# HKUST-Aerial-Robotics/FUEL

Hardware: AMD Instinct MI355X
Metric: plan_cycles_per_sec (higher is better)
Workload: dtype u64 bit-planes / u16 (u32 beyond 255 voxels) exact squared distances / f32 ESDF / f64 log-odds and B-spline

## Files before the change

fuel_amd/_lib.py:

```python
import ctypes as C
import os

_HERE = os.path.dirname(os.path.abspath(__file__))
LIB_PATH = os.environ.get("FUELMI_LIB_PATH") or os.path.join(_HERE, "libfuelmi.so")
_LIB = None

K_INFLATE, K_ESDF_ZY, K_ESDF_X, K_FRONTIER, K_BSPLINE, K_INSERT, K_COUNT = range(7)


class FuelmiError(RuntimeError):
    pass


class MapCfg(C.Structure):
    _fields_ = [
        ("resolution", C.c_double),
        ("map_size", C.c_double * 3),
        ("ground_height", C.c_double),
        ("obstacles_inflation", C.c_double),
        ("local_bound_inflate", C.c_double),
        ("default_dist", C.c_double),
        ("optimistic", C.c_int),
        ("signed_dist", C.c_int),
        ("p_hit", C.c_double),
# ... 264 lines not shown
    "fuelmi_map_get_updated_box": (C.c_int, [_P, _dp, _dp, C.c_int]),
    "fuelmi_map_set_updated_box": (C.c_int, [_P, _dp, _dp]),
    "fuelmi_map_upload_occupancy": (C.c_int, [_P, _dp]),
    "fuelmi_map_sync_host": (C.c_int, [_P, _ip, _ip, _dp, C.c_void_p, _dp]),
    "fuelmi_map_register_mirrors": (C.c_int, [_P, _dp, C.c_void_p, _dp]),
    "fuelmi_map_unregister_mirrors": (C.c_int, [_P]),
    "fuelmi_map_dist_grad": (C.c_int, [_P, _dp, C.c_int, _dp, _dp]),
    "fuelmi_map_coarse_dist": (C.c_int, [_P, _dp, C.c_int, _dp]),
    "fuelmi_map_query_state": (C.c_int, [_P, _ip, C.c_int, _ip, _ip]),
    "fuelmi_map_synchronize": (C.c_int, [_P]),
    "fuelmi_frontier_set_viewpoint_cfg": (C.c_int, [_P, C.POINTER(ViewpointCfg)]),
    "fuelmi_frontier_compute_to_visit": (C.c_int, [_P, C.POINTER(C.c_int), C.POINTER(C.c_int)]),
    "fuelmi_frontier_viewpoint_count": (C.c_int, [_P, C.c_int, C.c_int]),
    "fuelmi_frontier_viewpoints": (C.c_int, [_P, C.c_int, C.c_int, _dp, C.POINTER(C.c_int)]),
    "fuelmi_frontier_is_covered": (C.c_int, [_P, C.POINTER(C.c_int)]),
    "fuelmi_frontier_cluster_filtered_size": (C.c_int, [_P, C.c_int, C.c_int]),
    "fuelmi_frontier_cluster_filtered": (C.c_int, [_P, C.c_int, C.c_int, C.c_void_p]),
    "fuelmi_frontier_create": (C.c_int, [_P, C.POINTER(FrontierCfg), _PP]),
    "fuelmi_frontier_destroy": (None, [_P]),
    "fuelmi_frontier_reset": (C.c_int, [_P]),
    "fuelmi_frontier_stats": (C.c_int, [_P, C.POINTER(C.c_int)]),
    "fuelmi_frontier_resolved_in_launch": (C.c_int, [_P]),
    "fuelmi_frontier_path_stats": (C.c_int, [_P, C.POINTER(C.c_int)]),
    "fuelmi_frontier_changed_stats": (C.c_int, [_P, C.POINTER(C.c_int)]),
    "fuelmi_frontier_order_stats": (C.c_int, [_P, C.POINTER(C.c_int)]),
    "fuelmi_frontier_synchronize": (C.c_int, [_P]),
    "fuelmi_bench_cycles": (C.c_int, [_P, _P, _P, _dp, _dp, C.c_int, C.c_int, C.POINTER(C.c_int), _dp]),
    "fuelmi_bench_host_profile": (C.c_int, [_P, _dp]),
    "fuelmi_bench_cycles_delivered": (C.c_int, [_P, _P, _P, _dp, _dp, C.c_int, _ip, C.c_size_t, _dp, _dp,
                                                C.POINTER(C.c_int), _dp]),
    "fuelmi_bench_stream": (C.c_int, [_P, _P, _P, C.c_int, C.POINTER(C.c_void_p), C.c_int, C.c_int, C.POINTER(DepthCfg),
                                      _dp, _dp, C.c_int, C.POINTER(C.c_int), _dp, _dp]),
    "fuelmi_frontier_search": (C.c_int, [_P, _ip]),
    "fuelmi_frontier_search_begin": (C.c_int, [_P]),
    "fuelmi_frontier_search_end": (C.c_int, [_P, _ip]),
    "fuelmi_frontier_keep_previous": (C.c_int, [_P, C.c_int]),
    "fuelmi_frontier_commit": (C.c_int, [_P, C.c_int]),
    "fuelmi_frontier_count": (C.c_int, [_P, C.c_int]),
    "fuelmi_frontier_cluster_size": (C.c_int, [_P, C.c_int, C.c_int]),
    "fuelmi_frontier_cluster_cells": (C.c_int, [_P, C.c_int, C.c_int, _ip]),
    "fuelmi_frontier_cluster_centres": (C.c_int, [_P, C.c_int, C.c_int, _dp]),
    "fuelmi_frontier_cluster_info": (C.c_int, [_P, C.c_int, C.c_int, _dp]),
    "fuelmi_frontier_removed_count": (C.c_int, [_P]),
    "fuelmi_frontier_removed_ids": (C.c_int, [_P, _ip]),
    "fuelmi_frontier_get_flags": (C.c_int, [_P, C.c_void_p]),
    "fuelmi_map_path_costs": (C.c_int, [_P, C.POINTER(PathCfg), C.c_int, _dp, _dp, _dp, _ip, _ip, _dp]),
# ... 110 lines not shown
```

fuel_amd/csrc/frontier.hip:

```cpp
#include <algorithm>
#include <chrono>
#include <cmath>
#include <cstdlib>
#include <cstring>
#include <list>
#include <memory>
#include <vector>

#include "fuelmi_internal.h"
#include "frontier_internal.h"

__global__ void k_zero_words(u64* p, int n) {
  for (int i = blockIdx.x * blockDim.x + threadIdx.x; i < n; i += gridDim.x * blockDim.x) p[i] = 0ull;
}

template <typename T>
static int dmalloc(fuelmi_frontier* f, T** p, size_t n) {
  void* d = nullptr;
  HIPCHK(hipMalloc(&d, std::max<size_t>(n, 1) * sizeof(T)));
  f->allocs.push_back(d);
  *p = (T*)d;
  const char* fp = reinterpret_cast<const char*>(p), *f0 = reinterpret_cast<const char*>(&f->F);
  if (fp >= f0 && fp < f0 + sizeof(FArgs))
    f->f_scratch.push_back({(size_t)(fp - f0), std::max<size_t>(n, 1) * sizeof(T)});
// ... 209 lines not shown
  F.h_counts = reinterpret_cast<u32*>(f->h_pin);
  F.h_rec = reinterpret_cast<KeptRec*>(F.h_counts + 16);
  F.h_part = reinterpret_cast<u32*>(F.h_rec + F.cap_kept);
  F.h_cells = F.h_part + ((size_t)F.cap_q / SZ_CH + 2) * 10;
  F.hcells_direct_max = FR_HCELLS_DIRECT;
  f->TY = 16;
  f->TX = std::max(1, std::min(8, (48 * 1024) / (f->TY * g.nz * 4)));
  const int qx = F.qbox.hi[0] - F.qbox.lo[0] + 1, qy = F.qbox.hi[1] - F.qbox.lo[1] + 1;
  f->ccl_tiles = 0;
  if (qx > 0 && qy > 0 && F.qbox.lo[2] <= F.qbox.hi[2]) {
    const int TX = f->TX, TY = f->TY;
    const int ntx = (qx + TX - 1) / TX, nty = (qy + TY - 1) / TY;
    f->ccl_tiles = ntx * nty;
    f->ccl_lds = ((size_t)TX * TY * g.nz + 2 * (size_t)TX * TY * ((g.nz + 31) / 32) + 2 * (size_t)TX) * sizeof(u32);
    if (f->ccl_lds > 160 * 1024) {
      fuelmi_set_error("frontier CCL tile of %d z-lines x %d voxels does not fit the LDS", TX * TY, g.nz);
      fuelmi_frontier_destroy(f);
      return FUELMI_ELIMIT;
    }
    if ((rc = frontier_legacy_attrs(f))) return rc;
    const int mtx = 4, mty = 8;
    f->fast_tiles = ((qx + 1 + mtx - 1) / mtx) * ((qy + 1 + mty - 1) / mty);
    F.pm_stride = (qx + 1 + mtx - 1) / mtx;
    if ((rc = dmalloc(f, &F.vlab, (size_t)g.N + 64)) || (rc = dmalloc(f, &F.tlab, (size_t)f->fast_tiles * FR_TCELL)) ||
        (rc = dmalloc(f, &F.t_base, (size_t)f->fast_tiles)) || (rc = dmalloc(f, &F.t_nroots, (size_t)f->fast_tiles)) ||
        (rc = dmalloc(f, &F.pm, (size_t)FR_KCAP * F.pm_stride))) {
      fuelmi_frontier_destroy(f);
      return rc;
    }
    const size_t seg_words = frontier_tile_lds(f, qx, qy);
    if ((rc = dmalloc(f, &F.tq, seg_words + 64)) || (rc = dmalloc(f, &F.ts, seg_words + 64))) {
      fuelmi_frontier_destroy(f);
      return rc;
    }
  }
  if ((rc = frontier_tile_attrs(f))) return rc;
  f->fast_ok = f->ccl_tiles > 0 && cfg->cluster_min >= 1 && frontier_tile_fits(f) && getenv("FUELMI_FRONTIER_LEGACY") == nullptr;
  if ((rc = frontier_twin_set(f))) {
    fuelmi_frontier_destroy(f);
    return rc;
  }
  {
    std::lock_guard<std::mutex> lk(m->dep_mu);
    m->dependents.push_back({f, &frontier_orphan});
  }
  *out = f;
  return FUELMI_OK;
}

int frontier_materialize_lists(fuelmi_frontier* f) {
  if (!f->lazy_kept) return FUELMI_OK;
  for (std::list<HCluster>* L : {&f->frontiers, &f->dormant})
    for (HCluster& c : *L)
      if (c.lazy) {
// ... 640 lines not shown
```

fuel_amd/csrc/frontier_internal.h:

```cpp
#ifndef FUELMI_FRONTIER_INTERNAL_H_
#define FUELMI_FRONTIER_INTERNAL_H_

#include <algorithm>
#include <chrono>
#include <cstring>
#include <list>
#include <memory>
#include <vector>

#include "fuelmi_internal.h"

#define NOCLAIM 0xFFFFFFFFu
#define SZ_CH 1024

struct KeptRec {
  u32 addr, slot, size, off;
  unsigned long long sum[3];
  u32 box[6];
  u32 pad[2];
};

struct FVar {
  Box3 sbox;
  int w0;
// ... 52 lines not shown
  u32* parent;
  u32* claim;
  int* cell_slot;
  u32* seed_adr;
  u32* csize;
  u32* kept;
  u32 cap_kept;
  int* slot2rank;
  struct KeptRec* krec;
  u32* ms_key[2];
  u32* ms_val[2];
  u32* ms_hist;
  u32 ms_nb_max;
  u32* info_part;
  u32* h_counts;
  struct KeptRec* h_rec;
  u32* h_part;
  u32* h_cells;
  u32 hcells_direct_max;
  int keys_from_slots;
  FVar* var_w;
  u32* tq;
  u32* ts;
  unsigned char* vlab;
  unsigned char* tlab;
  u32* t_base;
  u32* t_nroots;
  struct TRec* trec;
  u32* tclaim;
  u32* rcode;
  unsigned short* rrow;
  u32* pm;
  int pm_stride;
  u32* pairs;
  u32* fctr;
  int fast;
  unsigned long long* dbg;
};
#define FR_HCELLS_DIRECT 32768u
#define FR_DBG_SLOTS 16
#define FR_DBG_MARK(F, blk, k)                                                                   \
  do {                                                                                           \
    if ((F).dbg && threadIdx.x == 0) (F).dbg[(size_t)(blk) * FR_DBG_SLOTS + (k)] = wall_clock64(); \
  } while (0)

#ifdef __HIPCC__
__device__ __forceinline__ void st_agent(u32* p, u32 v) { __hip_atomic_store(p, v, __ATOMIC_RELAXED, __HIP_MEMORY_SCOPE_AGENT); }
// ... 36 lines not shown
    v = OP(v, dpp_mov<0x140, 0xF>(ID, v));  \
    v = OP(v, dpp_mov<0x142, 0xA>(ID, v));                \
    v = OP(v, dpp_mov<0x143, 0xC>(ID, v));                \
    return (u32)__builtin_amdgcn_readlane((int)v, 63);                                       \
  }
__device__ __forceinline__ u32 red_add_(u32 a, u32 b) { return a + b; }
__device__ __forceinline__ u32 red_min_(u32 a, u32 b) { return min(a, b); }
__device__ __forceinline__ u32 red_max_(u32 a, u32 b) { return max(a, b); }
FUELMI_WAVE_RED(wave_add_u32, red_add_, 0u)
FUELMI_WAVE_RED(wave_min_u32, red_min_, 0xFFFFFFFFu)
FUELMI_WAVE_RED(wave_max_u32, red_max_, 0u)

__device__ __forceinline__ u64 q_window34(const Geo& g, const FVar& V, const FArgs& F, int xx, int yy, int c) {
  const bool inside = xx >= V.px0 && xx <= V.px1 && yy >= V.py0 && yy <= V.py1;
  const int xc = min(max(xx, V.px0), V.px1), yc = min(max(yy, V.py0), V.py1);
  const int nseg = (g.nz + 31) >> 5;
  const int tx = (xc - V.px0) / V.ftx, ty = (yc - V.py0) / V.fty;
  const int lx = xc - V.px0 - tx * V.ftx, ly = yc - V.py0 - ty * V.fty;
  const u32* p = F.tq + (size_t)(tx * V.nty_f + ty) * (size_t)(V.ftx * V.fty * nseg) + (size_t)(lx * V.fty + ly) * nseg + c;
  const bool has_lo = c > 0, has_hi = c + 1 < nseg;
  const u32 lo = p[has_lo ? -1 : 0], mid = p[0], hi = p[has_hi ? 1 : 0];
  const u64 w = (u64)(has_lo ? lo >> 31 : 0u) | ((u64)mid << 1) | ((u64)(has_hi ? hi & 1u : 0u) << 33);
  return inside ? w : 0ull;
}

__device__ __forceinline__ u32 q_bits3(const Geo& g, const FVar& V, const FArgs& F, int xx, int yy, int z) {
  const int c = z >> 5;
  return (u32)(q_window34(g, V, F, xx, yy, c) >> (z - 32 * c)) & 7u;
}
__device__ __forceinline__ u32 rank_s(const FArgs& F, long a) {
  int w = (int)(a >> 6);
  int rel = w - F.var->w0;
  u64 pk = F.blockscan[rel >> 8] + F.pref[rel];
  return (u32)(pk >> 32) + (u32)__popcll(F.sb[w] & ((1ull << (a & 63)) - 1ull));
}

__device__ __forceinline__ u64 f1_word(const Geo& g, const u64* __restrict__ occ, const u64* __restrict__ unk,
                                       int w, u64 z0, u64 zl, u64 y0, u64 yl) {
  long a0 = 64L * w;
  u64 valid = (a0 + 64 <= g.N) ? ~0ull : bit_range(0, (int)max(0L, g.N - a0));
  u64 free_ = ~occ[w] & ~unk[w] & valid;
  if (free_ == 0ull) return 0ull;
  u64 nb = (plane_window(unk, a0 + 1) & ~zl) | (plane_window(unk, a0 - 1) & ~z0) |
           (plane_window(unk, a0 + g.nz) & ~yl) | (plane_window(unk, a0 - g.nz) & ~y0) |
           plane_window(unk, a0 + g.nyz) | plane_window(unk, a0 - g.nyz);
  return free_ & nb;
// ... 344 lines not shown
```

fuel_amd/csrc/frontier_tile.hip:

```cpp
#include <algorithm>
#include <cstdlib>

#include "frontier_internal.h"

struct TileGeo {
  int tx, ty, x0, y0, nxl, nyl, TX, TY, nseg, items;
};
struct TilePro {
  FVar V;
  u32 ovf, nroots, gbase, pad;
};
__device__ __forceinline__ void stage_tile_pro(const FArgs& F, TilePro* sp) {
  constexpr int NV = (int)(sizeof(FVar) / 4);
  static_assert(sizeof(FVar) % 4 == 0 && NV + 3 <= 64, "FVar does not fit one wave's lanes");
  const int t = threadIdx.x;
  const u32* src = reinterpret_cast<const u32*>(F.var) + (t < NV ? t : 0);
  if (t == NV) src = F.counts + 2;
  if (t == NV + 1) src = F.t_nroots + blockIdx.x;
  if (t == NV + 2) src = F.t_base + blockIdx.x;
  if (t < NV + 3) reinterpret_cast<u32*>(sp)[t] = *src;
  __syncthreads();
}
__device__ __forceinline__ TileGeo tile_geo(const Geo& g, const FVar& V, int t) {
  TileGeo T;
// ... 211 lines not shown
  const int nz = g.nz, nseg = T.nseg, items = T.items, TY = T.TY;
  u32* lab = reinterpret_cast<u32*>(smem_raw);
  u32* segb = lab + FR_TCELL;
  u32* segpre = segb + items;
  u32* acc = segpre + items + 1;
  u32* rrow = acc + FR_TROOT * 8;
  unsigned short* rootno = reinterpret_cast<unsigned short*>(rrow + FR_TROOT * FR_TXS);
  unsigned char* rcell = reinterpret_cast<unsigned char*>(rootno + FR_TCELL);
  u32* segs = reinterpret_cast<u32*>(rcell + FR_TCELL);
  u32* plist = reinterpret_cast<u32*>(rootno);
  unsigned short* cseg = reinterpret_cast<unsigned short*>(acc);
  static_assert((size_t)FR_TCELL * sizeof(unsigned short) <= (size_t)FR_TROOT * 8 * 4 + (size_t)FR_TROOT * FR_TXS * 4, "cell -> segment table does not fit");
  static_assert((size_t)FR_TPAIR * sizeof(u32) <= FR_TCELL * sizeof(unsigned short) + FR_TCELL, "pair list does not fit");
  __shared__ u32 s_wsum[NT / 64];
  __shared__ u32 s_nroots, s_base, s_flag;
  __shared__ u32 s_cnt[4];
  const int lane = threadIdx.x & 63;
  if (threadIdx.x == 0) s_nroots = 0u, s_flag = 0u, s_cnt[0] = s_cnt[1] = s_cnt[2] = s_cnt[3] = 0u;
  FR_DBG_MARK(F, blockIdx.x, 0);
  const u32 total = tile_load_pred<NT>(g, T, V, F, segb, segpre, s_wsum, lab, segs, cseg);
  {
    u32* tq = F.tq + (size_t)blockIdx.x * items;
    u32* ts = F.ts + (size_t)blockIdx.x * items;
    for (int it = threadIdx.x; it < items; it += NT) tq[it] = segb[it], ts[it] = segs[it];
  }
  FR_DBG_MARK(F, blockIdx.x, 1);
  if (total == 0u || total > FR_TCELL) {
    if (threadIdx.x == 0) {
      F.t_nroots[blockIdx.x] = 0u;
      F.t_base[blockIdx.x] = 0u;
      if (total > FR_TCELL) F.fctr[FCTR(9)] = 11u;
    }
    return;
  }
  FR_DBG_MARK(F, blockIdx.x, 2);
  __shared__ u32 s_np, s_chg, s_povf;
  if (threadIdx.x == 0) s_np = 0u, s_chg = 0u, s_povf = 0u;
  __syncthreads();
  auto walk_pairs = [&](auto&& fn) {
    for (u32 l = threadIdx.x; l < total; l += NT) {
      const int it = cseg[l];
      const u32 bits = segb[it];
      u32 k = l - segpre[it], rem = bits;
      while (k--) rem &= rem - 1u;
      const int zz = __builtin_ctz(rem);
      const int line = it / nseg, c = it - line * nseg, lx = line / TY, ly = line - lx * TY;
      const int z = 32 * c + zz;
// ... 196 lines not shown
    const u32* r = acc + threadIdx.x * 8;
    const u32* rw = rrow + threadIdx.x * FR_TXS;
    TRec R;
    u32 size = 0u, sx = 0u, lox = 0xFFFFFFFFu, hix = 0u;
    unsigned short* grow = F.rrow + (size_t)(gbase + threadIdx.x) * FR_TXS;
    for (int lx = 0; lx < FR_TXS; ++lx) {
      const u32 cnt = lx < T.TX ? rw[lx] : 0u;
      grow[lx] = (unsigned short)cnt;
      if (cnt) {
        size += cnt, sx += cnt * (u32)(T.x0 + lx);
        lox = min(lox, (u32)(T.x0 + lx)), hix = max(hix, (u32)(T.x0 + lx));
      }
    }
    R.size = size, R.sx = sx, R.sy = r[0], R.sz = r[1];
    R.lo[0] = lox, R.lo[1] = r[3], R.lo[2] = r[4], R.hi[0] = hix, R.hi[1] = r[5], R.hi[2] = r[6];
    R.tx = (u32)T.tx, R.own = r[2];
    F.trec[gbase + threadIdx.x] = R;
    F.tclaim[gbase + threadIdx.x] = r[2];
  }
  {
    unsigned char* tl = F.tlab + (size_t)blockIdx.x * FR_TCELL;
    for (u32 l = threadIdx.x; l < total; l += NT) tl[l] = rcell[l];
  }
  for (int it = threadIdx.x; it < items; it += NT) {
    u32 rem = segb[it];
    if (!rem) continue;
    const int line = it / nseg, c = it - line * nseg;
    unsigned char* vl = F.vlab + tile_line_adr(g, T, line) + 32 * c;
    u32 l = segpre[it];
    while (rem) {
      const int b = __builtin_ctz(rem);
      rem &= rem - 1u;
      vl[b] = rcell[l++];
    }
  }
  FR_DBG_MARK(F, blockIdx.x, 6);
  if (F.dbg && threadIdx.x == 0) {
    F.dbg[(size_t)blockIdx.x * FR_DBG_SLOTS + 8] = total;
    F.dbg[(size_t)blockIdx.x * FR_DBG_SLOTS + 9] = s_cnt[0];
    F.dbg[(size_t)blockIdx.x * FR_DBG_SLOTS + 10] = s_cnt[1];
    F.dbg[(size_t)blockIdx.x * FR_DBG_SLOTS + 11] = s_cnt[2];
    F.dbg[(size_t)blockIdx.x * FR_DBG_SLOTS + 12] = nroots;
  }
}

#define XC_SET 256
#define XC_WCAP 6144
template <int RS_T, bool IN_LAUNCH>
__device__ __forceinline__ bool resolve_body(const Geo& g, const FArgs& F, const FVar& V, unsigned char* smem_raw, const u32 rcap);

__device__ __forceinline__ void xc_insert(u32* s_set, u32* s_list, u32* s_n, u32* fctr, u32 key) {
  u32 h = (key * 2654435761u) >> 24;
  bool done = false;
  for (int probe = 0; probe < XC_SET && !done; ++probe) {
    const u32 old = atomicCAS(&s_set[h], 0xFFFFFFFFu, key);
    if (old == 0xFFFFFFFFu) {
      s_list[atomicAdd(s_n, 1u)] = key;
      done = true;
    } else if (old == key)
      done = true;
    h = (h + 1u) & (XC_SET - 1u);
  }
  if (!done) st_agent(&fctr[FCTR(9)], 15u);
}
template <int NT>
__global__ void __launch_bounds__(NT) k_tile_cross(Geo g, FArgs F, const u32 rcap) {
  FR_DBG_MARK(F, blockIdx.x, 13);
  __shared__ TilePro s_pro;
  stage_tile_pro(F, &s_pro);
  const FVar& V = s_pro.V;
  if ((int)blockIdx.x >= V.ntiles_f) return;
  const TileGeo T = tile_geo(g, V, blockIdx.x);
  const int nz = g.nz, nseg = T.nseg, TY = T.TY;
  const int lane = threadIdx.x & 63;
  extern __shared__ __attribute__((aligned(16))) unsigned char smem_raw[];
  u32* segq = reinterpret_cast<u32*>(smem_raw);
  u32* segs = segq + T.items;
  u32* wl = segs + T.items;
  __shared__ u32 s_set[XC_SET];
  __shared__ u32 s_list[XC_SET];
  __shared__ u32 s_n, s_base, s_nw;
  __shared__ u32 s_tb[9];
  const int dblk = V.ntiles_f + 1 + (int)blockIdx.x;
  FR_DBG_MARK(F, dblk, 0);
  u32 tb9;
  {
    const int t9 = (int)threadIdx.x % 9, dtx = t9 / 3 - 1, dty = t9 % 3 - 1;
    const int ntx = T.tx + dtx, nty = T.ty + dty;
    const bool ok = ntx >= 0 && ntx < V.ntx_f && nty >= 0 && nty < V.nty_f;
    tb9 = F.t_base[ok ? ntx * V.nty_f + nty : (int)blockIdx.x];
    if (!ok) tb9 = 0u;
  }
  if (threadIdx.x < XC_SET) s_set[threadIdx.x] = 0xFFFFFFFFu;
  if (threadIdx.x == 0) s_n = 0u, s_nw = 0u;
  tile_load_arrays<NT, false>(T, F, segq, nullptr, nullptr, segs);
  if (threadIdx.x < 9) s_tb[threadIdx.x] = tb9;
  FR_DBG_MARK(F, dblk, 1);
  auto tile_of = [&](int x, int y) -> u32 {
    const int dtx = x < T.x0 ? -1 : (x >= T.x0 + T.TX ? 1 : 0), dty = y < T.y0 ? -1 : (y >= T.y0 + TY ? 1 : 0);
    return (u32)((dtx + 1) * 3 + dty + 1);
  };
  u32 k0 = 0xFFFFFFFFu, k1 = 0xFFFFFFFFu;
  auto do_item = [&](u32 bits, u32 own, int nb, u32 info, u64 w3) {
    const int c = (int)(info & 0xFFu);
    const u32 tb = s_tb[(info >> 8) & 0xFFu];
    w3 &= (1ull << 34) - 1ull;
    if (c == 0) w3 &= ~1ull;
    const int jend = nz - 32 * c + 1;
    if (jend < 34) w3 &= (1ull << jend) - 1ull;
    if (info >> 16) {
      while (w3) {
        int j, rl;
        pop_run64(w3, j, rl);
        const int b0 = max(j - 2, 0), b1 = min(j + rl - 1, 31);
        if (b0 > b1) continue;
        const u32 m = bits & (((b1 - b0 + 1 >= 32) ? 0xFFFFFFFFu : ((1u << (b1 - b0 + 1)) - 1u)) << b0);
        if (!m) continue;
        const u32 r = tb + (u32)F.vlab[(long)nb + j];
        atomicMin(&F.tclaim[r], own + (u32)__builtin_ctz(m));
      }
      return;
    }
    u32 rem = bits;
    while (rem && w3) {
      int s, len;
      pop_run32(rem, s, len);
      u64 m = (w3 >> s) & ((1ull << (len + 2)) - 1ull);
      if (!m) continue;
      const u32 ga = s_tb[4] + (u32)F.vlab[(long)own + s];
      while (m) {
        int j, rl;
        pop_run64(m, j, rl);
        const u32 gb = tb + (u32)F.vlab[(long)nb + s + j];
        if (gb == ga) continue;
        const u32 key = (min(ga, gb) << 16) | max(ga, gb);
        if (key == k0 || key == k1) continue;
        if (k0 == 0xFFFFFFFFu)
          k0 = key;
        else if (k1 == 0xFFFFFFFFu)
          k1 = key;
        else
          xc_insert(s_set, s_list, &s_n, F.fctr, key);
      }
    }
  };
  auto flush_pairs = [&]() {
#pragma unroll
    for (int q = 0; q < 2; ++q) {
      const u32 kq = q ? k1 : k0;
      const bool on = kq != 0xFFFFFFFFu;
      u64 todo = __ballot(on);
      while (todo) {
        const int leader = __builtin_ctzll(todo);
        const u32 key = (u32)__shfl((int)kq, leader, 64);
        todo &= ~__ballot(on && kq == key);
        if (lane == leader) xc_insert(s_set, s_list, &s_n, F.fctr, key);
      }
    }
    k0 = k1 = 0xFFFFFFFFu;
  };
  auto decode = [&](u32 e, u32& bits, u32& own, int& nb, u32& info, int& xx, int& yy) {
    int it, c;
    if (e >> 31) {
      const int sj = (int)(e & 0x7FFFFFFFu), l = sj % 9;
      it = sj / 9;
      const int line = it / nseg, lx = line / TY, ly = line - lx * TY;
      c = it - line * nseg;
      xx = T.x0 + lx + l / 3 - 1, yy = T.y0 + ly + l % 3 - 1;
      bits = (xx >= V.px0 && xx <= V.px1 && yy >= V.py0 && yy <= V.py1) ? segs[it] : 0u;
      own = (u32)((long)(T.x0 + lx) * g.nyz + (long)(T.y0 + ly) * nz + 32 * c);
      info = (u32)c | (tile_of(xx, yy) << 8) | (1u << 16);
    } else {
      const int k = (int)(e & 3u), fs = (int)(e >> 2), fl = fs / nseg;
      c = fs - fl * nseg;
      int lx = 0, ly = fl;
      if (fl >= TY) lx = 1 + ((fl - TY) >> 1), ly = ((fl - TY) & 1) ? TY - 1 : 0;
      xx = T.x0 + lx + (k < 3 ? -1 : 0), yy = T.y0 + ly + (k < 3 ? k - 1 : -1);
      bits = segq[(lx * TY + ly) * nseg + c];
      own = (u32)((long)(T.x0 + lx) * g.nyz + (long)(T.y0 + ly) * nz + 32 * c);
      info = (u32)c | (tile_of(xx, yy) << 8);
    }
    nb = (int)((long)xx * g.nyz + (long)yy * nz + 32 * c - 1);
  };
  const int nfl = TY + 2 * (T.nxl - 1);
  const int fitems = nfl * nseg * 4;
  for (int fi = threadIdx.x; fi < fitems; fi += NT) {
    const int k = fi & 3, fs = fi >> 2, fl = fs / nseg, c = fs - fl * nseg;
    int lx = 0, ly = fl;
    if (fl >= TY) lx = 1 + ((fl - TY) >> 1), ly = ((fl - TY) & 1) ? TY - 1 : 0;
    if (!segq[(lx * TY + ly) * nseg + c]) continue;
    const int kdx = k < 3 ? -1 : 0, kdy = k < 3 ? k - 1 : -1;
    const int xx = T.x0 + lx + kdx, yy = T.y0 + ly + kdy;
    const bool cross = (kdx < 0 && lx == 0) || (kdy < 0 && ly == 0) || (kdy > 0 && ly == TY - 1);
    if (!(cross && ly < T.nyl && xx >= V.px0 && yy >= V.py0 && yy <= V.py1)) continue;
    const u32 slot = atomicAdd(&s_nw, 1u);
    if (slot < XC_WCAP)
      wl[slot] = (u32)fi;
    else
      st_agent(&F.fctr[FCTR(9)], 18u);
  }
  for (int it = threadIdx.x; it < T.items; it += NT) {
    if (!segs[it]) continue;
    const u32 slot0 = atomicAdd(&s_nw, 9u);
    for (int l = 0; l < 9; ++l) {
      const u32 e = 0x80000000u | (u32)(it * 9 + l);
      if (slot0 + (u32)l < XC_WCAP)
        wl[slot0 + (u32)l] = e;
      else
        st_agent(&F.fctr[FCTR(9)], 18u);
    }
  }
  __syncthreads();
  FR_DBG_MARK(F, dblk, 2);
  const u32 nw = min(s_nw, (u32)XC_WCAP);
  for (u32 w0 = 0; w0 < nw; w0 += 2 * NT) {
    u32 b0 = 0u, b1 = 0u, o0 = 0u, o1 = 0u, i0 = 0u, i1 = 0u;
    int n0 = 0, n1 = 0, xa = 0, ya = 0, xb = 0, yb = 0;
    u64 wa = 0ull, wb = 0ull;
    const u32 ja = w0 + threadIdx.x, jb = ja + NT;
    if (ja < nw) decode(wl[ja], b0, o0, n0, i0, xa, ya);
    if (jb < nw) decode(wl[jb], b1, o1, n1, i1, xb, yb);
    wa = q_window34(g, V, F, xa, ya, (int)(i0 & 0xFFu));
    wb = q_window34(g, V, F, xb, yb, (int)(i1 & 0xFFu));
    if (!b0) wa = 0ull;
    if (!b1) wb = 0ull;
#pragma nounroll
    for (int h = 0; h < 2; ++h) {
      const u32 bb = h ? b1 : b0;
      const u64 ww = h ? wb : wa;
      if (bb && ww) do_item(bb, h ? o1 : o0, h ? n1 : n0, h ? i1 : i0, ww);
      flush_pairs();
    }
  }
  __syncthreads();
  FR_DBG_MARK(F, dblk, 3);
  const u32 n = s_n;
  if (n != 0u) {
    const u32 xcd = blockIdx.x & 7u;
    if (threadIdx.x == 0) s_base = atomicAdd(&F.fctr[FCTR(16 + xcd)], n);
    __syncthreads();
    const u32 base = s_base;
    if (base + n > FR_PCAP / 8u) {
      if (threadIdx.x == 0) st_agent(&F.fctr[FCTR(9)], 14u);
    } else if (threadIdx.x < n)
      st_agent(&F.pairs[(size_t)xcd * (FR_PCAP / 8u) + base + threadIdx.x], s_list[threadIdx.x]);
  }
// ... 565 lines not shown
      if (ckey[l++] != 0xFFFFu) fl |= 1u << b;
    }
    if (!fl) continue;
    const int line = it / nseg, c = it - line * nseg;
    or_flags(tile_line_adr(g, T, line) + 32 * c, fl);
  }  FR_DBG_MARK(F, dblk, 6);
}

static const int kFastMenu[4][2] = {{16, 32}, {8, 32}, {8, 16}, {4, 8}};
int menu_tiles(int qx, int qy, int mk) {
  return ((qx + kFastMenu[mk][0] - 1) / kFastMenu[mk][0]) * ((qy + kFastMenu[mk][1] - 1) / kFastMenu[mk][1]);
}
static int fast_launch_tiles(const FArgs& F, int mk) {
  return menu_tiles(F.qbox.hi[0] - F.qbox.lo[0] + 2, F.qbox.hi[1] - F.qbox.lo[1] + 2, mk);
}
void set_fast_tiles(FVar& hv, int mk) {
  const int qx = hv.px1 - hv.px0 + 1, qy = hv.py1 - hv.py0 + 1;
  hv.ftx = kFastMenu[mk][0], hv.fty = kFastMenu[mk][1];
  hv.ntx_f = std::max(0, (qx + hv.ftx - 1) / hv.ftx);
  hv.nty_f = std::max(0, (qy + hv.fty - 1) / hv.fty);
  hv.ntiles_f = hv.ntx_f * hv.nty_f;
}

int frontier_enqueue_fast(fuelmi_frontier* f) {
  const Geo& g = f->map->g;
  FArgs& F = f->F;
  const int mk = f->fast_menu;
  const int tiles = fast_launch_tiles(F, mk);
  if (f->tl_ev) HIPCHK(hipEventRecord(f->tl_ev[0], f->stream));
  k_tile_ccl<512><<<tiles, 512, f->tile_lds[mk], f->stream>>>(g, F, *f->h_var);
  FDBG("k_tile_ccl");
  g_ht.lap(4);
  if (f->mark_planes_read) {
    HIPCHK(hipEventRecord(f->ev_planes_read, f->stream));
    map_add_plane_reader(f->map, f->ev_planes_read);
  } else {
    map_add_late_reader(f->map, f->stream, f->ev_planes_read, &f->mark_planes_read);
  }
  if (f->tl_ev) HIPCHK(hipEventRecord(f->tl_ev[1], f->stream));
  g_ht.lap(5);
  {
    bool fuse_now = f->h_var->ntiles_f > 0;
    if (fuse_now && f->fuse_skip > 0) --f->fuse_skip, fuse_now = false;
    f->fuse_tried = fuse_now;
    const size_t lds_x = fuse_now ? std::max(f->cross_lds[mk], resolve_lds_bytes(1024)) : f->cross_lds[mk];
    const u32 rcap = fuse_now ? (u32)std::min<size_t>((lds_x - resolve_lds_bytes(0)) / 16, FR_RCAP) : 0u;
// ... 5 lines not shown
  g_ht.lap(6);
  if (f->kr_queued) k_resolve<<<1, RS_TK, f->resolve_lds, f->stream>>>(g, F);
  FDBG("k_resolve");
  g_ht.lap(7);
  if (f->tl_ev) HIPCHK(hipEventRecord(f->tl_ev[2], f->stream));
  k_tile_out<512><<<tiles, 512, f->out_lds[mk], f->stream>>>(g, F);
  FDBG("k_tile_out");
  g_ht.lap(8);
  if (f->tl_ev) HIPCHK(hipEventRecord(f->tl_ev[3], f->stream));
  HIPCHK(hipGetLastError());
  return FUELMI_OK;
}

size_t frontier_tile_lds(fuelmi_frontier* f, int qx, int qy) {
  const Geo& g = f->map->g;
  size_t seg_words = 0;
  for (int k = 0; k < 4; ++k) {
    const int ftx = kFastMenu[k][0], fty = kFastMenu[k][1];
    const size_t items = (size_t)(ftx * fty) * ((g.nz + 31) / 32);
    seg_words = std::max(seg_words, (size_t)((qx + 1 + ftx - 1) / ftx) * ((qy + 1 + fty - 1) / fty) * items);
    f->fast_items[k] = items;
    f->tile_lds[k] = (FR_TCELL + 3 * items + 1 + (size_t)FR_TROOT * 8 + (size_t)FR_TROOT * FR_TXS) * sizeof(u32) +
                     FR_TCELL * sizeof(unsigned short) + FR_TCELL;
    f->cross_lds[k] = (2 * items + (size_t)XC_WCAP) * sizeof(u32);
    f->out_lds[k] = (3 * items + 1 + FR_TCELL + 2 * (size_t)kFastMenu[k][0] * FR_TROOT + FR_KCAP + FR_TROOT) * sizeof(u32) +
                    FR_TCELL * sizeof(unsigned short);
    f->tile_lds[k] = (f->tile_lds[k] + 15) & ~(size_t)15;
    f->cross_lds[k] = (f->cross_lds[k] + 15) & ~(size_t)15;
    f->out_lds[k] = (f->out_lds[k] + 15) & ~(size_t)15;
  }
  return seg_words;
}
int frontier_tile_attrs(fuelmi_frontier* f) {
  const size_t lds_max = std::max(f->tile_lds[0], f->out_lds[0]);
  if (lds_max > 64 * 1024 && lds_max <= 150 * 1024) {
    HIPCHK(hipFuncSetAttribute(reinterpret_cast<const void*>(&k_tile_ccl<512>), hipFuncAttributeMaxDynamicSharedMemorySize, 150 * 1024));
    HIPCHK(hipFuncSetAttribute(reinterpret_cast<const void*>(&k_tile_out<512>), hipFuncAttributeMaxDynamicSharedMemorySize, 150 * 1024));
  }
  f->resolve_lds = resolve_lds_bytes(FR_RCAP);
  HIPCHK(hipFuncSetAttribute(reinterpret_cast<const void*>(&k_resolve), hipFuncAttributeMaxDynamicSharedMemorySize,
                             (int)f->resolve_lds));
  return FUELMI_OK;
}
bool frontier_tile_fits(const fuelmi_frontier* f) {
  return std::max(f->tile_lds[0], f->out_lds[0]) <= 150 * 1024 && f->fast_items[0] <= (size_t)FT_PER * 512;
}

int frontier_enqueue_late_resolve(fuelmi_frontier* f) {
  const Geo& g = f->map->g;
  FArgs& F = f->F;
  const int mk = f->fast_menu;
  k_resolve<<<1, RS_TK, f->resolve_lds, f->stream>>>(g, F);
  k_tile_out<512><<<fast_launch_tiles(F, mk), 512, f->out_lds[mk], f->stream>>>(g, F);
  HIPCHK(hipGetLastError());
  return FUELMI_OK;
}
// ... 1 lines not shown
```

fuel_amd/host.py:

```python
import ctypes as C

import numpy as np

from . import _lib
from ._lib import (BsplineBatch, BsplineCfg, CloudCfg, ColRangeCfg, FrontierCfg, GainCfg, GoalCfg, KinoCfg, LocalSegCfg, MapCfg, MapInfo, PathCfg, RefineCfg, RenderCfg, TopoCfg, TrajAdjCfg, TrajChkCfg, TrajSmpCfg, TspCfg,
                   WptrajCfg, YawCfg, YawPathCfg, check, lib)

DEFAULT_MAP = dict(resolution=0.1, ground_height=-1.0, obstacles_inflation=0.199,
                   local_bound_inflate=0.5, default_dist=0.0, optimistic=0, signed_dist=0,
                   p_hit=0.65, p_miss=0.35, p_min=0.12, p_max=0.90, p_occ=0.80,
                   max_ray_length=4.5, virtual_ceil_height=-10.0)
DEFAULT_BSPLINE = dict(ld_smooth=20.0, ld_dist=10.0, ld_feasi=2.0, ld_start=100.0, ld_end=0.5,
                       ld_guide=1.5, ld_waypt=0.3, ld_view=0.0, ld_time=1.0, dist0=0.7,
                       max_vel=2.0, max_acc=2.0, wnl=1.0, dlmin=0.0, bspline_degree=3)

SMOOTHNESS, DISTANCE, FEASIBILITY, START, END, GUIDE, WAYPOINTS, VIEWCONS, MINTIME = \
    (1 << k for k in range(9))
GUIDE_PHASE = SMOOTHNESS | GUIDE | START | END
NORMAL_PHASE = SMOOTHNESS | DISTANCE | FEASIBILITY | START | END


def _dp(a):
    return None if a is None else a.ctypes.data_as(C.POINTER(C.c_double))

# ... 1182 lines not shown
        return n.value

    def commit(self, dormant=False):
        check(self.L.fuelmi_frontier_commit(self.h, int(dormant)))

    def reset(self):
        check(self.L.fuelmi_frontier_reset(self.h))

    def sync(self):
        from ._lib import check as _c
        _c(self.L.fuelmi_frontier_synchronize(self.h))

    def stats(self):
        o = (C.c_int * 3)()
        check(self.L.fuelmi_frontier_stats(self.h, o))
        return tuple(o)

    def resolvedInLaunch(self):
        return self.L.fuelmi_frontier_resolved_in_launch(self.h)

    def pathStats(self):
        o = (C.c_int * 2)()
        check(self.L.fuelmi_frontier_path_stats(self.h, o))
        return tuple(o)

    def changedStats(self):
        o = (C.c_int * 9)()
        check(self.L.fuelmi_frontier_changed_stats(self.h, o))
        return {"paths": tuple(o[:4]), "nc": o[4], "total": o[5], "mark": o[6], "rebuilds": o[7], "pool_cap": o[8]}

    def orderStats(self):
        o = (C.c_int * 4)()
        check(self.L.fuelmi_frontier_order_stats(self.h, o))
        return tuple(o)

    def clusters(self, which=0):
        out = []
        cnt = self.L.fuelmi_frontier_count(self.h, which)
        if cnt < 0:
            check(cnt)
        for k in range(cnt):
            n = self.L.fuelmi_frontier_cluster_size(self.h, which, k)
            a = np.empty(n, dtype=np.int32)
            check(self.L.fuelmi_frontier_cluster_cells(self.h, which, k, _ip(a)))
            out.append(a)
        return out
# ... 354 lines not shown
```

include/fuelmi.h:

```cpp
#ifndef FUELMI_H_
#define FUELMI_H_

#include <stddef.h>
#include <stdint.h>

#ifdef __cplusplus
extern "C" {
#endif

#define FUELMI_OK 0
#define FUELMI_EINVAL (-1)
#define FUELMI_ENODEV (-2)
#define FUELMI_EHIP (-3)
#define FUELMI_ENOMEM (-4)
#define FUELMI_ELIMIT (-5)

#define FUELMI_HWQ_UNINIT 0
#define FUELMI_HWQ_SET 1
#define FUELMI_HWQ_ENV 2
#define FUELMI_HWQ_LATE 3
int fuelmi_init(int hw_queues);
int fuelmi_hw_queues(void);
int fuelmi_hw_queues_state(void);
const char* fuelmi_last_error(void);
// ... 91 lines not shown
int fuelmi_map_dist_grad(fuelmi_map* m, const double* pos_xyz, int n, double* dist, double* grad_xyz);
int fuelmi_map_coarse_dist(fuelmi_map* m, const double* pos_xyz, int n, double* dist);
int fuelmi_map_query_state(fuelmi_map* m, const int* idx_xyz, int n, int* occupancy, int* inflate);

int fuelmi_map_synchronize(fuelmi_map* m);

typedef struct {
  int cluster_min;
  double min_z;
  double cluster_size_xy;
  int down_sample;
  int split;
  int reference_order;
} fuelmi_frontier_cfg;

typedef struct fuelmi_frontier fuelmi_frontier;

int fuelmi_frontier_create(fuelmi_map* m, const fuelmi_frontier_cfg* cfg, fuelmi_frontier** out);
void fuelmi_frontier_destroy(fuelmi_frontier* f);
int fuelmi_frontier_reset(fuelmi_frontier* f);
int fuelmi_frontier_stats(const fuelmi_frontier* f, int out3[3]);
int fuelmi_frontier_resolved_in_launch(const fuelmi_frontier* f);
int fuelmi_frontier_path_stats(const fuelmi_frontier* f, int out2[2]);
int fuelmi_frontier_changed_stats(const fuelmi_frontier* f, int out[9]);
int fuelmi_frontier_order_stats(const fuelmi_frontier* f, int out4[4]);
int fuelmi_frontier_synchronize(fuelmi_frontier* f);
typedef struct {
  double candidate_rmin, candidate_rmax;
  int candidate_rnum;
  double candidate_dphi;
  double min_candidate_clearance;
  int min_visib_num;
  double min_candidate_dist;
  double min_view_finish_fraction;
  double top_angle, left_angle, right_angle, max_dist;
} fuelmi_viewpoint_cfg;
int fuelmi_frontier_set_viewpoint_cfg(fuelmi_frontier* f, const fuelmi_viewpoint_cfg* cfg);
int fuelmi_frontier_compute_to_visit(fuelmi_frontier* f, int* n_active_new, int* n_dormant_new);
int fuelmi_frontier_viewpoint_count(const fuelmi_frontier* f, int which, int k);
int fuelmi_frontier_viewpoints(const fuelmi_frontier* f, int which, int k, double* pos_yaw4, int* visib);
int fuelmi_frontier_is_covered(fuelmi_frontier* f, int* covered);
int fuelmi_frontier_cluster_filtered_size(const fuelmi_frontier* f, int which, int k);
int fuelmi_frontier_cluster_filtered(const fuelmi_frontier* f, int which, int k, float* xyz);
int fuelmi_frontier_search(fuelmi_frontier* f, int* n_new);
int fuelmi_frontier_search_begin(fuelmi_frontier* f);
int fuelmi_frontier_search_end(fuelmi_frontier* f, int* n_new);
// ... 503 lines not shown
```

Baseline: 11260.

## Replace dense per-voxel label map with compact per-tile labels and prefix counts

Removes the full-grid vlab byte map that the CCL kernel scattered labels into. It now stores a per-segment prefix-count array (tpre), and the cross-tile merge kernel recovers labels by indexing the compact per-tile tlab with popcount. The own-tile labels and prefixes are staged in LDS. This drops a scattered full-grid write and random global reads, at the cost of extra popcount arithmetic, an extra tpre store, and more LDS in the cross kernel. A small tile-shape query API is also added.

```diff
diff --git a/fuel_amd/_lib.py b/fuel_amd/_lib.py
--- a/fuel_amd/_lib.py
+++ b/fuel_amd/_lib.py
@@ -310,6 +310,7 @@
     "fuelmi_frontier_stats": (C.c_int, [_P, C.POINTER(C.c_int)]),
     "fuelmi_frontier_resolved_in_launch": (C.c_int, [_P]),
     "fuelmi_frontier_path_stats": (C.c_int, [_P, C.POINTER(C.c_int)]),
+    "fuelmi_frontier_tile_shape": (C.c_int, [_P, C.POINTER(C.c_int)]),
     "fuelmi_frontier_changed_stats": (C.c_int, [_P, C.POINTER(C.c_int)]),
     "fuelmi_frontier_order_stats": (C.c_int, [_P, C.POINTER(C.c_int)]),
     "fuelmi_frontier_synchronize": (C.c_int, [_P]),
diff --git a/fuel_amd/csrc/frontier.hip b/fuel_amd/csrc/frontier.hip
--- a/fuel_amd/csrc/frontier.hip
+++ b/fuel_amd/csrc/frontier.hip
@@ -255,14 +255,15 @@
     const int mtx = 4, mty = 8;
     f->fast_tiles = ((qx + 1 + mtx - 1) / mtx) * ((qy + 1 + mty - 1) / mty);
     F.pm_stride = (qx + 1 + mtx - 1) / mtx;
-    if ((rc = dmalloc(f, &F.vlab, (size_t)g.N + 64)) || (rc = dmalloc(f, &F.tlab, (size_t)f->fast_tiles * FR_TCELL)) ||
+    if ((rc = dmalloc(f, &F.tlab, (size_t)f->fast_tiles * FR_TCELL)) ||
         (rc = dmalloc(f, &F.t_base, (size_t)f->fast_tiles)) || (rc = dmalloc(f, &F.t_nroots, (size_t)f->fast_tiles)) ||
         (rc = dmalloc(f, &F.pm, (size_t)FR_KCAP * F.pm_stride))) {
       fuelmi_frontier_destroy(f);
       return rc;
     }
     const size_t seg_words = frontier_tile_lds(f, qx, qy);
-    if ((rc = dmalloc(f, &F.tq, seg_words + 64)) || (rc = dmalloc(f, &F.ts, seg_words + 64))) {
+    if ((rc = dmalloc(f, &F.tq, seg_words + 64)) || (rc = dmalloc(f, &F.ts, seg_words + 64)) ||
+        (rc = dmalloc(f, &F.tpre, seg_words + 64))) {
       fuelmi_frontier_destroy(f);
       return rc;
     }
diff --git a/fuel_amd/csrc/frontier_internal.h b/fuel_amd/csrc/frontier_internal.h
--- a/fuel_amd/csrc/frontier_internal.h
+++ b/fuel_amd/csrc/frontier_internal.h
@@ -98,7 +98,7 @@
   FVar* var_w;
   u32* tq;
   u32* ts;
-  unsigned char* vlab;
+  unsigned short* tpre;
   unsigned char* tlab;
   u32* t_base;
   u32* t_nroots;
@@ -181,6 +181,30 @@
   const u32 lo = p[has_lo ? -1 : 0], mid = p[0], hi = p[has_hi ? 1 : 0];
   const u64 w = (u64)(has_lo ? lo >> 31 : 0u) | ((u64)mid << 1) | ((u64)(has_hi ? hi & 1u : 0u) << 33);
   return inside ? w : 0ull;
+}
+
+__device__ __forceinline__ u64 q_window34p(const Geo& g, const FVar& V, const FArgs& F, int xx, int yy, int c, u32& row) {
+  const bool inside = xx >= V.px0 && xx <= V.px1 && yy >= V.py0 && yy <= V.py1;
+  const int xc = min(max(xx, V.px0), V.px1), yc = min(max(yy, V.py0), V.py1);
+  const int nseg = (g.nz + 31) >> 5;
+  const int tx = (xc - V.px0) / V.ftx, ty = (yc - V.py0) / V.fty;
+  const int lx = xc - V.px0 - tx * V.ftx, ly = yc - V.py0 - ty * V.fty;
+  const int tile = tx * V.nty_f + ty;
+  const size_t at = (size_t)tile * (size_t)(V.ftx * V.fty * nseg) + (size_t)(lx * V.fty + ly) * nseg + c;
+  const u32* p = F.tq + at;
+  const bool has_lo = c > 0, has_hi = c + 1 < nseg;
+  const u32 lo = p[has_lo ? -1 : 0], mid = p[0], hi = p[has_hi ? 1 : 0];
+  const u32 pre = (u32)F.tpre[at];
+  const u64 w = (u64)(has_lo ? lo >> 31 : 0u) | ((u64)mid << 1) | ((u64)(has_hi ? hi & 1u : 0u) << 33);
+  const u32 b0 = (u32)(w & 1ull);
+  row = (u32)tile * FR_TCELL + min(pre > b0 ? pre - b0 : 0u, (u32)(FR_TCELL - 1));
+  return inside ? w : 0ull;
+}
+__device__ __forceinline__ u32 tlab_at(const FArgs& F, u32 row, u64 wr, int j) {
+  static_assert((FR_TCELL & (FR_TCELL - 1)) == 0, "the tile of a tlab entry is its index / FR_TCELL");
+  const u32 i = row + (u32)__popcll(wr & ((1ull << j) - 1ull));
+  const u32 t0 = row & ~(u32)(FR_TCELL - 1);
+  return (u32)F.tlab[(size_t)t0 + min(i - t0, (u32)(FR_TCELL - 1))];
 }
 
 __device__ __forceinline__ u32 q_bits3(const Geo& g, const FVar& V, const FArgs& F, int xx, int yy, int z) {
diff --git a/fuel_amd/csrc/frontier_tile.hip b/fuel_amd/csrc/frontier_tile.hip
--- a/fuel_amd/csrc/frontier_tile.hip
+++ b/fuel_amd/csrc/frontier_tile.hip
@@ -257,7 +257,9 @@
   {
     u32* tq = F.tq + (size_t)blockIdx.x * items;
     u32* ts = F.ts + (size_t)blockIdx.x * items;
-    for (int it = threadIdx.x; it < items; it += NT) tq[it] = segb[it], ts[it] = segs[it];
+    unsigned short* tp = F.tpre + (size_t)blockIdx.x * items;
+    for (int it = threadIdx.x; it < items; it += NT)
+      tq[it] = segb[it], ts[it] = segs[it], tp[it] = (unsigned short)min(segpre[it], 0xFFFFu);
   }
   FR_DBG_MARK(F, blockIdx.x, 1);
   if (total == 0u || total > FR_TCELL) {
@@ -500,18 +502,6 @@
     unsigned char* tl = F.tlab + (size_t)blockIdx.x * FR_TCELL;
     for (u32 l = threadIdx.x; l < total; l += NT) tl[l] = rcell[l];
   }
-  for (int it = threadIdx.x; it < items; it += NT) {
-    u32 rem = segb[it];
-    if (!rem) continue;
-    const int line = it / nseg, c = it - line * nseg;
-    unsigned char* vl = F.vlab + tile_line_adr(g, T, line) + 32 * c;
-    u32 l = segpre[it];
-    while (rem) {
-      const int b = __builtin_ctz(rem);
-      rem &= rem - 1u;
-      vl[b] = rcell[l++];
-    }
-  }
   FR_DBG_MARK(F, blockIdx.x, 6);
   if (F.dbg && threadIdx.x == 0) {
     F.dbg[(size_t)blockIdx.x * FR_DBG_SLOTS + 8] = total;
@@ -555,6 +545,8 @@
   u32* segq = reinterpret_cast<u32*>(smem_raw);
   u32* segs = segq + T.items;
   u32* wl = segs + T.items;
+  unsigned short* spre = reinterpret_cast<unsigned short*>(wl + XC_WCAP);
+  unsigned char* slab = reinterpret_cast<unsigned char*>(spre + ((T.items + 1) & ~1));
   __shared__ u32 s_set[XC_SET];
   __shared__ u32 s_list[XC_SET];
   __shared__ u32 s_n, s_base, s_nw;
@@ -569,23 +561,50 @@
     tb9 = F.t_base[ok ? ntx * V.nty_f + nty : (int)blockIdx.x];
     if (!ok) tb9 = 0u;
   }
+  constexpr int XL_PER = (FR_TCELL / 4 + NT - 1) / NT, XP_PER = (FT_PER * NT / 2 + NT - 1) / NT;
+  u32 olab[XL_PER], opre[XP_PER];
+  {
+    const u32* tl = reinterpret_cast<const u32*>(F.tlab + (size_t)blockIdx.x * FR_TCELL);
+    const u32* tp = reinterpret_cast<const u32*>(F.tpre + (size_t)blockIdx.x * T.items);
+#pragma unroll
+    for (int k = 0; k < XL_PER; ++k) {
+      const int i = (int)threadIdx.x + k * NT;
+      olab[k] = i < FR_TCELL / 4 ? tl[i] : 0u;
+    }
+#pragma unroll
+    for (int k = 0; k < XP_PER; ++k) {
+      const int i = (int)threadIdx.x + k * NT;
+      opre[k] = i < T.items / 2 ? tp[i] : 0u;
+    }
+  }
   if (threadIdx.x < XC_SET) s_set[threadIdx.x] = 0xFFFFFFFFu;
   if (threadIdx.x == 0) s_n = 0u, s_nw = 0u;
   tile_load_arrays<NT, false>(T, F, segq, nullptr, nullptr, segs);
   if (threadIdx.x < 9) s_tb[threadIdx.x] = tb9;
+#pragma unroll
+  for (int k = 0; k < XL_PER; ++k) {
+    const int i = (int)threadIdx.x + k * NT;
+    if (i < FR_TCELL / 4) reinterpret_cast<u32*>(slab)[i] = olab[k];
+  }
+#pragma unroll
+  for (int k = 0; k < XP_PER; ++k) {
+    const int i = (int)threadIdx.x + k * NT;
+    if (i < T.items / 2) reinterpret_cast<u32*>(spre)[i] = opre[k];
+  }
   FR_DBG_MARK(F, dblk, 1);
   auto tile_of = [&](int x, int y) -> u32 {
     const int dtx = x < T.x0 ? -1 : (x >= T.x0 + T.TX ? 1 : 0), dty = y < T.y0 ? -1 : (y >= T.y0 + TY ? 1 : 0);
     return (u32)((dtx + 1) * 3 + dty + 1);
   };
   u32 k0 = 0xFFFFFFFFu, k1 = 0xFFFFFFFFu;
-  auto do_item = [&](u32 bits, u32 own, int nb, u32 info, u64 w3) {
+  auto do_item = [&](u32 bits, u32 own, u32 nrow, u32 info, u64 w3) {
     const int c = (int)(info & 0xFFu);
     const u32 tb = s_tb[(info >> 8) & 0xFFu];
     w3 &= (1ull << 34) - 1ull;
     if (c == 0) w3 &= ~1ull;
     const int jend = nz - 32 * c + 1;
     if (jend < 34) w3 &= (1ull << jend) - 1ull;
+    const u64 wr = w3;
     if (info >> 16) {
       while (w3) {
         int j, rl;
@@ -594,7 +613,7 @@
         if (b0 > b1) continue;
         const u32 m = bits & (((b1 - b0 + 1 >= 32) ? 0xFFFFFFFFu : ((1u << (b1 - b0 + 1)) - 1u)) << b0);
         if (!m) continue;
-        const u32 r = tb + (u32)F.vlab[(long)nb + j];
+        const u32 r = tb + tlab_at(F, nrow, wr, j);
         atomicMin(&F.tclaim[r], own + (u32)__builtin_ctz(m));
       }
       return;
@@ -605,11 +624,11 @@
       pop_run32(rem, s, len);
       u64 m = (w3 >> s) & ((1ull << (len + 2)) - 1ull);
       if (!m) continue;
-      const u32 ga = s_tb[4] + (u32)F.vlab[(long)own + s];
+      const u32 ga = s_tb[4] + (u32)slab[min((u32)spre[own] + (u32)__popc(bits & ((1u << s) - 1u)), (u32)(FR_TCELL - 1))];
       while (m) {
         int j, rl;
         pop_run64(m, j, rl);
-        const u32 gb = tb + (u32)F.vlab[(long)nb + s + j];
+        const u32 gb = tb + tlab_at(F, nrow, wr, s + j);
         if (gb == ga) continue;
         const u32 key = (min(ga, gb) << 16) | max(ga, gb);
         if (key == k0 || key == k1) continue;
@@ -637,7 +656,7 @@
     }
     k0 = k1 = 0xFFFFFFFFu;
   };
-  auto decode = [&](u32 e, u32& bits, u32& own, int& nb, u32& info, int& xx, int& yy) {
+  auto decode = [&](u32 e, u32& bits, u32& own, u32& info, int& xx, int& yy) {
     int it, c;
     if (e >> 31) {
       const int sj = (int)(e & 0x7FFFFFFFu), l = sj % 9;
@@ -654,11 +673,10 @@
       int lx = 0, ly = fl;
       if (fl >= TY) lx = 1 + ((fl - TY) >> 1), ly = ((fl - TY) & 1) ? TY - 1 : 0;
       xx = T.x0 + lx + (k < 3 ? -1 : 0), yy = T.y0 + ly + (k < 3 ? k - 1 : -1);
-      bits = segq[(lx * TY + ly) * nseg + c];
-      own = (u32)((long)(T.x0 + lx) * g.nyz + (long)(T.y0 + ly) * nz + 32 * c);
+      own = (u32)((lx * TY + ly) * nseg + c);
+      bits = segq[own];
       info = (u32)c | (tile_of(xx, yy) << 8);
     }
-    nb = (int)((long)xx * g.nyz + (long)yy * nz + 32 * c - 1);
   };
   const int nfl = TY + 2 * (T.nxl - 1);
   const int fitems = nfl * nseg * 4;
@@ -692,14 +710,14 @@
   FR_DBG_MARK(F, dblk, 2);
   const u32 nw = min(s_nw, (u32)XC_WCAP);
   for (u32 w0 = 0; w0 < nw; w0 += 2 * NT) {
-    u32 b0 = 0u, b1 = 0u, o0 = 0u, o1 = 0u, i0 = 0u, i1 = 0u;
-    int n0 = 0, n1 = 0, xa = 0, ya = 0, xb = 0, yb = 0;
+    u32 b0 = 0u, b1 = 0u, o0 = 0u, o1 = 0u, i0 = 0u, i1 = 0u, n0 = 0u, n1 = 0u;
+    int xa = 0, ya = 0, xb = 0, yb = 0;
     u64 wa = 0ull, wb = 0ull;
     const u32 ja = w0 + threadIdx.x, jb = ja + NT;
-    if (ja < nw) decode(wl[ja], b0, o0, n0, i0, xa, ya);
-    if (jb < nw) decode(wl[jb], b1, o1, n1, i1, xb, yb);
-    wa = q_window34(g, V, F, xa, ya, (int)(i0 & 0xFFu));
-    wb = q_window34(g, V, F, xb, yb, (int)(i1 & 0xFFu));
+    if (ja < nw) decode(wl[ja], b0, o0, i0, xa, ya);
+    if (jb < nw) decode(wl[jb], b1, o1, i1, xb, yb);
+    wa = q_window34p(g, V, F, xa, ya, (int)(i0 & 0xFFu), n0);
+    wb = q_window34p(g, V, F, xb, yb, (int)(i1 & 0xFFu), n1);
     if (!b0) wa = 0ull;
     if (!b1) wb = 0ull;
 #pragma nounroll
@@ -1311,6 +1329,13 @@
   hv.ntiles_f = hv.ntx_f * hv.nty_f;
 }
 
+extern "C" int fuelmi_frontier_tile_shape(const fuelmi_frontier* f, int out2[2]) {
+  ARGCHK(f && out2);
+  const bool fast = f->F.fast != 0 && f->n_fast > 0;
+  out2[0] = fast ? kFastMenu[f->fast_menu][0] : 0, out2[1] = fast ? kFastMenu[f->fast_menu][1] : 0;
+  return FUELMI_OK;
+}
+
 int frontier_enqueue_fast(fuelmi_frontier* f) {
   const Geo& g = f->map->g;
   FArgs& F = f->F;
@@ -1362,7 +1387,7 @@
     f->fast_items[k] = items;
     f->tile_lds[k] = (FR_TCELL + 3 * items + 1 + (size_t)FR_TROOT * 8 + (size_t)FR_TROOT * FR_TXS) * sizeof(u32) +
                      FR_TCELL * sizeof(unsigned short) + FR_TCELL;
-    f->cross_lds[k] = (2 * items + (size_t)XC_WCAP) * sizeof(u32);
+    f->cross_lds[k] = (2 * items + (size_t)XC_WCAP) * sizeof(u32) + ((items + 1) & ~(size_t)1) * sizeof(unsigned short) + FR_TCELL;
     f->out_lds[k] = (3 * items + 1 + FR_TCELL + 2 * (size_t)kFastMenu[k][0] * FR_TROOT + FR_KCAP + FR_TROOT) * sizeof(u32) +
                     FR_TCELL * sizeof(unsigned short);
     f->tile_lds[k] = (f->tile_lds[k] + 15) & ~(size_t)15;
@@ -1372,6 +1397,8 @@
   return seg_words;
 }
 int frontier_tile_attrs(fuelmi_frontier* f) {
+  if (f->cross_lds[0] > 64 * 1024 && f->cross_lds[0] <= 150 * 1024)
+    HIPCHK(hipFuncSetAttribute(reinterpret_cast<const void*>(&k_tile_cross<512>), hipFuncAttributeMaxDynamicSharedMemorySize, 150 * 1024));
   const size_t lds_max = std::max(f->tile_lds[0], f->out_lds[0]);
   if (lds_max > 64 * 1024 && lds_max <= 150 * 1024) {
     HIPCHK(hipFuncSetAttribute(reinterpret_cast<const void*>(&k_tile_ccl<512>), hipFuncAttributeMaxDynamicSharedMemorySize, 150 * 1024));
diff --git a/fuel_amd/host.py b/fuel_amd/host.py
--- a/fuel_amd/host.py
+++ b/fuel_amd/host.py
@@ -1228,6 +1228,11 @@
     def pathStats(self):
         o = (C.c_int * 2)()
         check(self.L.fuelmi_frontier_path_stats(self.h, o))
+        return tuple(o)
+
+    def tileShape(self):
+        o = (C.c_int * 2)()
+        check(self.L.fuelmi_frontier_tile_shape(self.h, o))
         return tuple(o)
 
     def changedStats(self):
diff --git a/include/fuelmi.h b/include/fuelmi.h
--- a/include/fuelmi.h
+++ b/include/fuelmi.h
@@ -137,6 +137,7 @@
 int fuelmi_frontier_stats(const fuelmi_frontier* f, int out3[3]);
 int fuelmi_frontier_resolved_in_launch(const fuelmi_frontier* f);
 int fuelmi_frontier_path_stats(const fuelmi_frontier* f, int out2[2]);
+int fuelmi_frontier_tile_shape(const fuelmi_frontier* f, int out2[2]);
 int fuelmi_frontier_changed_stats(const fuelmi_frontier* f, int out[9]);
 int fuelmi_frontier_order_stats(const fuelmi_frontier* f, int out4[4]);
 int fuelmi_frontier_synchronize(fuelmi_frontier* f);
```

Result: no change. 11450 (median of 6 runs) (+1.7%).
